# lionelblonde/sac-td3-cudagraphs-pytorch

Hardware: AMD Instinct MI355X
Metric: gradient-steps/sec (SAC, batch=256) at 1 GPU + 8-seed node; replay HBM GB/s (higher is better)
Workload: dtype f32; 1 GPU; SAC Hopper-v4 batch=256 2x256 MLP+LN, 100000 rows in a 1000000-row HBM ring, 1 critic update+Polyak per iteration, 2 actor+alpha updates every 3rd, hipGraph per 3 iterations; parallelism=1 independent seeds, one per GPU, no collective

## Files before the change

sac-td3-cudagraphs-pytorch_amd/csrc/kernels.h:

```cpp
#pragma once
#include <hip/hip_runtime.h>
#include <stddef.h>
#include <stdint.h>
#include <type_traits>
#include "philox.h"

#define HID 256
#define LN_EPS 1e-5f
#define NSLOT 5
#define AS 260
#define WS 68
#define YS 20

typedef float f32x4 __attribute__((ext_vector_type(4)));

#ifdef SACTD3_STAMPS
__device__ long long g_stamps[16];
__device__ long long g_phase[8];
#define PHASE_DECL long long ph_t = 0, ph_acc[6] = {0, 0, 0, 0, 0, 0}
#define PHASE_START do { __builtin_amdgcn_s_waitcnt(0xc07f); ph_t = clock64(); } while (0)
#define PHASE(i) do { const long long n_ = clock64(); ph_acc[i] += n_ - ph_t; ph_t = n_; } while (0)
#define PHASE_DRAIN(i) do { __builtin_amdgcn_s_waitcnt(0); const long long n_ = clock64(); ph_acc[i] += n_ - ph_t; ph_t = n_; } while (0)
#define PHASE_OUT do { if (threadIdx.x == 0 && blockIdx.x == gridDim.x - 1) for (int i_ = 0; i_ < 6; ++i_) g_phase[i_] = ph_acc[i_]; } while (0)
#define STAMP(i) do { if (threadIdx.x == 0 && blockIdx.x == gridDim.x - 1 && blockIdx.y == 0 && blockIdx.z == 0) { __builtin_amdgcn_s_waitcnt(0); g_stamps[i] = clock64(); } } while (0)
// ... 29 lines not shown
  int pad_seq;
  float metrics[8];
  float adam_q[2], adam_a[2];
  double pw_q[2], pw_a[2], pw_l[2];
  alignas(128) int predict_ctr;
  int predict_seq;
  int pad_acting[30];
};
static_assert(offsetof(DevCtl, predict_ctr) % 128 == 0 && sizeof(DevCtl) % 128 == 0, "acting words need a line of their own");

struct NetLayout {
  int K, ld1, nh;
  int W1, b1, g1, be1, W2, b2, g2, be2, Wh, bh;
  int size;
};

__device__ __forceinline__ unsigned fast_div(unsigned n, unsigned d, unsigned magic) { return magic ? __umulhi(n, magic) : n / d; }
__device__ __forceinline__ int small_div(int n, int d) {
  int q = (int)((float)n * __frcp_rn((float)d));
  const int r = n - q * d;
  if (r < 0) --q; else if (r >= d) ++q;
  return q;
}
__device__ __forceinline__ void xcd_tile(int b, int R, int C, int xr, int& tr, int& tc) {
  if (xr <= 0) { tr = small_div(b, C); tc = b - tr * C; return; }
  const int lr = __builtin_ctz((unsigned)xr), lc = 3 - lr;
  const int x = b & 7, j = b >> 3;
  const int cl = C >> lc, rl = R >> lr;
  const int gr = x >> lc, gc = x - (gr << lc);
  const int jr = small_div(j, cl);
  tr = gr * rl + jr; tc = gc * cl + (j - jr * cl);
}

__device__ __forceinline__ void adam_tick(int* t, double* pw, float* out, float lr, float b1, float b2) {
  const int tv = *t;
  double q0 = 0.0, q1 = 0.0;
  if (out) { q0 = pw[0]; q1 = pw[1]; }
  *t = tv + 1;
  if (out) {
    const double p1 = q0 * (double)b1, p2 = q1 * (double)b2;
    pw[0] = p1; pw[1] = p2;
    out[0] = (float)((double)lr / (1.0 - p1));
    out[1] = (float)sqrt(1.0 - p2);
  }
}
__device__ int g_sink_i[2];
__device__ double g_sink_d[2];
__device__ float g_sink_f[2];
__device__ __forceinline__ void tick_all(int* t0, int* t1, double* pw, float* out, float lr, float b1, float b2) {
  const bool pub = t0 != nullptr && out != nullptr;
  t0 = t0 ? t0 : g_sink_i; t1 = t1 ? t1 : g_sink_i + 1;
  pw = pub ? pw : g_sink_d; out = pub ? out : g_sink_f;
  const int a = *t0, b = *t1;
  const double q0 = pw[0], q1 = pw[1];
  const double p1 = q0 * (double)b1, p2 = q1 * (double)b2;
  *t0 = a + 1; *t1 = b + 1;
  pw[0] = p1; pw[1] = p2;
  out[0] = (float)((double)lr / (1.0 - p1));
  out[1] = (float)sqrt(1.0 - p2);
}
#define PIN(x) asm volatile("" : "+v"(x))
template <int CTRL> __device__ __forceinline__ float dpp_mov(float v) {
  return __builtin_bit_cast(float, __builtin_amdgcn_update_dpp(0, __builtin_bit_cast(int, v), CTRL, 0xF, 0xF, true));
}
__device__ __forceinline__ float row16_sum(float v) {
  v += dpp_mov<0xB1>(v);
  v += dpp_mov<0x4E>(v);
  v += dpp_mov<0x141>(v);
  v += dpp_mov<0x140>(v);
  return v;
}
__device__ __forceinline__ float lane_bcast(float v, int l) {
  return __builtin_bit_cast(float, __builtin_amdgcn_readlane(__builtin_bit_cast(int, v), l));
}
__device__ __forceinline__ float wave_sum(float v) {
  v = row16_sum(v);
  return (lane_bcast(v, 0) + lane_bcast(v, 16)) + (lane_bcast(v, 32) + lane_bcast(v, 48));
}
__device__ __forceinline__ float sum4(float4 v) { return (v.x + v.y) + (v.z + v.w); }
__device__ __forceinline__ float dot4(float4 a, float4 b) { return a.x * b.x + a.y * b.y + a.z * b.z + a.w * b.w; }
__device__ __forceinline__ float4 ld4(const float* p) { return *reinterpret_cast<const float4*>(p); }
__device__ __forceinline__ void st4(float* p, float4 v) { *reinterpret_cast<float4*>(p) = v; }
#ifndef SACTD3_WT
#define SACTD3_WT 1
#endif
constexpr bool WT_ACT1 = (SACTD3_WT & 1) != 0;
constexpr bool WT_Z2 = (SACTD3_WT & 2) != 0;
constexpr bool WT_DZ = (SACTD3_WT & 4) != 0;
typedef unsigned int u32x4 __attribute__((ext_vector_type(4)));
__device__ __forceinline__ void st4_wt(float* base, long off, float4 v) {
  const u32x4 u = {__float_as_uint(v.x), __float_as_uint(v.y), __float_as_uint(v.z), __float_as_uint(v.w)};
  __builtin_amdgcn_raw_buffer_store_b128(u, __builtin_amdgcn_make_buffer_rsrc(base, 0, 0x7fffffff, 0x00020000), (int)(4 * off), 0, 16);
}
__device__ __forceinline__ void st1_wt(float* p, float v) { __hip_atomic_store(p, v, __ATOMIC_RELAXED, __HIP_MEMORY_SCOPE_AGENT); }
template <bool WT> __device__ __forceinline__ void st4_pol(float* base, long off, float4 v) { if (WT) st4_wt(base, off, v); else st4(base + off, v); }
template <bool WT> __device__ __forceinline__ void st1_pol(float* p, float v) { if (WT) st1_wt(p, v); else *p = v; }
__device__ __forceinline__ float4 f4(float a) { return make_float4(a, a, a, a); }
__device__ __forceinline__ float4 operator+(float4 a, float4 b) { return make_float4(a.x + b.x, a.y + b.y, a.z + b.z, a.w + b.w); }
__device__ __forceinline__ float4 operator-(float4 a, float4 b) { return make_float4(a.x - b.x, a.y - b.y, a.z - b.z, a.w - b.w); }
__device__ __forceinline__ float4 operator*(float4 a, float4 b) { return make_float4(a.x * b.x, a.y * b.y, a.z * b.z, a.w * b.w); }
__device__ __forceinline__ float4 operator*(float4 a, float b) { return make_float4(a.x * b, a.y * b, a.z * b, a.w * b); }
__device__ __forceinline__ float4 relu4(float4 a) { return make_float4(fmaxf(a.x, 0.f), fmaxf(a.y, 0.f), fmaxf(a.z, 0.f), fmaxf(a.w, 0.f)); }
__device__ __forceinline__ float4 gate4(float4 v, float4 y) {
  return make_float4(y.x > 0.f ? v.x : 0.f, y.y > 0.f ? v.y : 0.f, y.z > 0.f ? v.z : 0.f, y.w > 0.f ? v.w : 0.f);
}
__device__ __forceinline__ float4 ld4_cols(const float* row, int k, int K, int Kr, bool row_ok = true) {
  const float4 v = ld4(row + min(k, Kr - 4));
  float4 o;
  o.x = (row_ok && k < K) ? v.x : 0.f;
  o.y = (row_ok && k + 1 < K) ? v.y : 0.f;
  o.z = (row_ok && k + 2 < K) ? v.z : 0.f;
  o.w = (row_ok && k + 3 < K) ? v.w : 0.f;
  return o;
}

__device__ __forceinline__ float4 ld4_raw(const float* row, int k, int Kr) { return ld4(row + min(k, Kr - 4)); }
__device__ __forceinline__ float4 mask4_cols(float4 v, int k, int K, bool row_ok = true) {
  float4 o;
  o.x = (row_ok && k < K) ? v.x : 0.f;
  o.y = (row_ok && k + 1 < K) ? v.y : 0.f;
  o.z = (row_ok && k + 2 < K) ? v.z : 0.f;
  o.w = (row_ok && k + 3 < K) ? v.w : 0.f;
  return o;
}

__device__ __forceinline__ float philox_normal(unsigned long long seed, unsigned ctr, unsigned site, unsigned e) {
  const Philox4 r = philox4x32_10(ctr, 0u, SACTD3_STREAM_NOISE + site, e >> 2, (uint32_t)seed, (uint32_t)(seed >> 32));
  const unsigned k = e & 3u;
  const float u1 = philox_u01((k & 2u) ? r.v[2] : r.v[0]), u2 = philox_u01((k & 2u) ? r.v[3] : r.v[1]);
  const float rad = sqrtf(-2.0f * 0.6931471805599453f * __builtin_amdgcn_logf(u1));
  return (k & 1u) ? rad * __builtin_amdgcn_sinf(u2) : rad * __builtin_amdgcn_cosf(u2);
}

__device__ __forceinline__ float4 philox_normal4(unsigned long long seed, unsigned ctr, unsigned site, unsigned q) {
  const Philox4 r = philox4x32_10(ctr, 0u, SACTD3_STREAM_NOISE + site, q, (uint32_t)seed, (uint32_t)(seed >> 32));
  const float ua = philox_u01(r.v[0]), ub = philox_u01(r.v[1]), uc = philox_u01(r.v[2]), ud = philox_u01(r.v[3]);
  const float r0 = sqrtf(-2.0f * 0.6931471805599453f * __builtin_amdgcn_logf(ua));
  const float r1 = sqrtf(-2.0f * 0.6931471805599453f * __builtin_amdgcn_logf(uc));
  return make_float4(r0 * __builtin_amdgcn_cosf(ub), r0 * __builtin_amdgcn_sinf(ub), r1 * __builtin_amdgcn_cosf(ud), r1 * __builtin_amdgcn_sinf(ud));
}
struct NoiseJob { float* eps; const int* ctr; int ctr_add; unsigned site_code; int site_buf; int n; int blocks; };
__device__ __forceinline__ void noise_body(const NoiseJob& z, const DevCtl* ctl, unsigned local_block) {
  const int inject = ctl->inject_eps[z.site_buf], ctr = *z.ctr;
  const unsigned long long seed = ctl->seed;
  const unsigned q = local_block * 256u + threadIdx.x;
  if (inject || 4 * q >= (unsigned)z.n) return;
  const float4 v = philox_normal4(seed, (unsigned)(ctr + z.ctr_add), z.site_code, q);
  float* d = z.eps + 4 * (long)q;
  d[0] = v.x;
  if (4 * q + 1 < (unsigned)z.n) d[1] = v.y;
  if (4 * q + 2 < (unsigned)z.n) d[2] = v.z;
  if (4 * q + 3 < (unsigned)z.n) d[3] = v.w;
}

struct Row16 { float4 v[4]; };
__device__ __forceinline__ Row16 row_ld(const float* row, int sub) {
  Row16 r;
#pragma unroll
  for (int q = 0; q < 4; ++q) r.v[q] = ld4(row + 4 * sub + 64 * q);
  return r;
}
__device__ __forceinline__ void row_pin(Row16& r) {
#pragma unroll
  for (int q = 0; q < 4; ++q) { PIN(r.v[q].x); PIN(r.v[q].y); PIN(r.v[q].z); PIN(r.v[q].w); }
}
__device__ __forceinline__ void row_st(float* row, int sub, const Row16& r) {
#pragma unroll
  for (int q = 0; q < 4; ++q) st4(row + 4 * sub + 64 * q, r.v[q]);
}
__device__ __forceinline__ float row_dot(const Row16& a, const Row16& b) {
  return (dot4(a.v[0], b.v[0]) + dot4(a.v[1], b.v[1])) + (dot4(a.v[2], b.v[2]) + dot4(a.v[3], b.v[3]));
}
__device__ __forceinline__ float row_total(const Row16& a) { return (sum4(a.v[0]) + sum4(a.v[1])) + (sum4(a.v[2]) + sum4(a.v[3])); }

__device__ __forceinline__ void ln_fwd(const Row16& z, const Row16& g, const Row16& be, int ln, Row16& xh, Row16& y, float& rstd) {
  if (ln) {
    const float mean = row16_sum(row_total(z)) * (1.0f / HID);
    Row16 d;
#pragma unroll
    for (int q = 0; q < 4; ++q) d.v[q] = z.v[q] - f4(mean);
    const float var = row16_sum(row_dot(d, d)) * (1.0f / HID);
    rstd = 1.0f / sqrtf(var + LN_EPS);
#pragma unroll
    for (int q = 0; q < 4; ++q) { xh.v[q] = d.v[q] * rstd; y.v[q] = xh.v[q] * g.v[q] + be.v[q]; }
  } else {
    rstd = 1.f; xh = z; y = z;
  }
}
__device__ __forceinline__ Row16 ln_bwd(const Row16& dy, const Row16& xh, float rstd, const Row16& g, int ln) {
  if (!ln) return dy;
  Row16 dxh, dz;
#pragma unroll
  for (int q = 0; q < 4; ++q) dxh.v[q] = dy.v[q] * g.v[q];
  const float m1 = row16_sum(row_total(dxh)) * (1.0f / HID);
  const float m2 = row16_sum(row_dot(dxh, xh)) * (1.0f / HID);
#pragma unroll
  for (int q = 0; q < 4; ++q) dz.v[q] = (dxh.v[q] - f4(m1) - xh.v[q] * m2) * rstd;
  return dz;
}
template <int RPB>
__device__ __forceinline__ void block_colsum(float* cs, const Row16* vals, int nslots, int row, int sub, float* dst) {
  for (int s = 0; s < nslots; ++s) row_st(cs + (s * RPB + row) * HID, sub, vals[s]);
  __syncthreads();
  for (int c = threadIdx.x; c < HID; c += 16 * RPB)
    for (int s = 0; s < nslots; ++s) {
      float a = 0.f;
#pragma unroll
      for (int r = 0; r < RPB; ++r) a += cs[(s * RPB + r) * HID + c];
      dst[s * HID + c] = a;
    }
}

struct GatherArgs {
  const float4* ring; int rec4;
  int cx, cn;
  const DevCtl* ctl; int* idx;
  float4* X; float4* Xn;
  float* rew; float* done;
  int B; int len_override;
  unsigned rec4_magic;
  int cpb;
  int ctr_add;
};

#ifndef GATHER_CPT
#define GATHER_CPT 4
#endif
__device__ __forceinline__ void gather_body(const GatherArgs& p, unsigned block) {
  __shared__ int ids_s[GATHER_CPT * 256 + 2];
  const int inject = p.ctl->inject_idx, rb_len = p.ctl->rb_len, ctr = p.ctl->sample_ctr + p.ctr_add;
  const unsigned long long seed = p.ctl->seed;
  const int len = p.len_override >= 0 ? p.len_override : rb_len;
  const unsigned total = (unsigned)p.B * (unsigned)p.rec4;
  const unsigned c0 = block * (unsigned)p.cpb * 256u;
  if (c0 >= total) return;
  const unsigned c1 = min(c0 + (unsigned)p.cpb * 256u, total);
// ... 1816 lines not shown
  const Row16 zo = row_ld(p.z2 + ((long)net * p.B + bc) * HID, sub);
  const Row16 wt0 = row_ld(p.PT + p.L.Wh, sub), wt1 = row_ld(p.PT + p.p_ns + p.L.Wh, sub), wo = row_ld(Pn + p.L.Wh, sub);
  Row16 gt0, bt0, gt1, bt1, go, bo;
  if (p.ln) {
    gt0 = row_ld(p.PT + p.L.g2, sub); bt0 = row_ld(p.PT + p.L.be2, sub);
    gt1 = row_ld(p.PT + p.p_ns + p.L.g2, sub); bt1 = row_ld(p.PT + p.p_ns + p.L.be2, sub);
    go = row_ld(Pn + p.L.g2, sub); bo = row_ld(Pn + p.L.be2, sub);
  }
  const float bht0 = p.PT[p.L.bh], bht1 = p.PT[p.p_ns + p.L.bh], bho = Pn[p.L.bh];
  const float rw = p.rew[bc], dn = p.done[bc];
  const float alpha = p.sac ? expf(*p.log_alpha) : 0.f;
  const float lpn = p.sac ? p.logp_next[bc] : 0.f;
  STAMP(1);
  Row16 xh, y, h; float rs;
  ln_fwd(zt0, gt0, bt0, p.ln, xh, y, rs);
#pragma unroll
  for (int q = 0; q < 4; ++q) h.v[q] = relu4(y.v[q]);
  const float qt0 = row16_sum(row_dot(h, wt0)) + bht0;
  ln_fwd(zt1, gt1, bt1, p.ln, xh, y, rs);
#pragma unroll
  for (int q = 0; q < 4; ++q) h.v[q] = relu4(y.v[q]);
  const float qt1 = row16_sum(row_dot(h, wt1)) + bht1;
  const float qmin = fminf(qt0, qt1);
  float qp = p.bcq ? 0.75f * qmin + 0.25f * fmaxf(qt0, qt1) : qmin;
  if (p.sac) qp -= alpha * lpn;
  const float yv = rw + (1.0f - dn) * p.gamma * qp;
  float rstd;
  ln_fwd(zo, go, bo, p.ln, xh, y, rstd);
#pragma unroll
  for (int q = 0; q < 4; ++q) h.v[q] = relu4(y.v[q]);
  const float qv = row16_sum(row_dot(h, wo)) + bho;
  const float err = valid ? qv - yv : 0.f;
  const float dq = 2.0f * err / (float)p.B;
  Row16 dy, vals[3];
#pragma unroll
  for (int q = 0; q < 4; ++q) dy.v[q] = gate4(wo.v[q] * dq, y.v[q]);
  const Row16 dz = ln_bwd(dy, xh, rstd, go, p.ln);
#pragma unroll
  for (int q = 0; q < 4; ++q) { vals[0].v[q] = dy.v[q] * xh.v[q]; vals[1].v[q] = dy.v[q]; vals[2].v[q] = h.v[q] * dq; }
  if (valid) {
    row_st(p.dz2 + ((long)net * p.B + b) * HID, sub, dz);
    if (sub == 0) {
      p.q[(long)net * p.B + b] = qv;
      if (net == 0) { p.qt[b] = qt0; p.qt[p.B + b] = qt1; p.y[b] = yv; }
    }
  }
  if (sub == 0) { sc[row][0] = dq; sc[row][1] = err * err; }
  STAMP(2);
  const long blk = (long)net * p.pstride + blockIdx.x;
  block_colsum<RPB>(cs, vals, 3, row, sub, p.part + blk * NSLOT * HID);
  if (t < 2) {
    float s = 0.f;
#pragma unroll
    for (int i = 0; i < RPB; ++i) s += sc[i][t];
    p.part_s[blk * 2 + t] = s;
  }
  STAMP(3);
}

struct NnFold { int fold, ln; const float* h1; const float* xh1; int g1_off; float* ps; float* gsnap; };
struct CtailNn { CriticTail c; const float* Wt; int ldw; float* dX; int xr; NnFold f; };
__device__ __forceinline__ void nn_fold_store(const NnFold& f, const float* o, const float* hv, const float* xv, float gcol,
                                              float* x, float* ps, float* gsnap, int row0, int B, int col, int lane) {
  if (f.fold && f.ln && row0 == 0 && lane < 16) gsnap[col] = gcol;
#pragma unroll
  for (int i = 0; i < 4; ++i) {
    const int orow = row0 + 4 * (lane >> 4) + i;
    const float dy = f.fold ? (hv[i] > 0.f ? o[i] : 0.f) : o[i];
    if (orow < B) x[(long)orow * HID + col] = dy;
    if (f.fold && f.ln) {
      const float dxh = dy * gcol;
      const float s1 = row16_sum(dxh), s2 = row16_sum(dxh * xv[i]);
      if ((lane & 15) == 0 && orow < B) { ps[(long)orow * PS_W + (col >> 4)] = s1; ps[(long)orow * PS_W + 16 + (col >> 4)] = s2; }
    }
  }
}
template <int NT>
__global__ __launch_bounds__(256) void k_ctail_nn(CtailNn a) {
  const CriticTail& p = a.c;
  constexpr int CB = 16 * NT;
  __shared__ __attribute__((aligned(16))) float Dz[16 * AS];
  __shared__ __attribute__((aligned(16))) float cs[3 * 16 * CB];
  __shared__ __attribute__((aligned(16))) float red[NT * 4 * 64 * 4];
  __shared__ float sc[16][2];
  const int t = threadIdx.x, lane = t & 63, wave = t >> 6, row = t >> 4, sub = t & 15, net = blockIdx.z;
  const int r = lane & 15, kq = lane >> 4;
  int tm, tk;
  xcd_tile(blockIdx.x, (p.B + 15) >> 4, HID / CB, a.xr, tm, tk);
  const int b = tm * 16 + row, bc = min(b, p.B - 1), c_lo = tk * CB;
  const bool valid = b < p.B;
  const float* Pn = p.P + net * p.p_ns;
  const Row16 zt0 = row_ld(p.z2t + (long)bc * HID, sub), zt1 = row_ld(p.z2t + ((long)p.B + bc) * HID, sub);
  const Row16 zo = row_ld(p.z2 + ((long)net * p.B + bc) * HID, sub);
  const Row16 wt0 = row_ld(p.PT + p.L.Wh, sub), wt1 = row_ld(p.PT + p.p_ns + p.L.Wh, sub), wo = row_ld(Pn + p.L.Wh, sub);
  Row16 gt0, bt0, gt1, bt1, go, bo;
  if (p.ln) {
    gt0 = row_ld(p.PT + p.L.g2, sub); bt0 = row_ld(p.PT + p.L.be2, sub);
    gt1 = row_ld(p.PT + p.p_ns + p.L.g2, sub); bt1 = row_ld(p.PT + p.p_ns + p.L.be2, sub);
    go = row_ld(Pn + p.L.g2, sub); bo = row_ld(Pn + p.L.be2, sub);
  }
  const float bht0 = p.PT[p.L.bh], bht1 = p.PT[p.p_ns + p.L.bh], bho = Pn[p.L.bh];
  const float rw = p.rew[bc], dn = p.done[bc];
  const float alpha = p.sac ? expf(*p.log_alpha) : 0.f;
  const float lpn = p.sac ? p.logp_next[bc] : 0.f;
  const int nb = 64 * wave + 4 * kq;
  float4 bv[NT][4];
#pragma unroll
  for (int nt = 0; nt < NT; ++nt) {
    const float* Wc = a.Wt + net * p.p_ns + (long)nb * a.ldw + c_lo + 16 * nt + r;
#pragma unroll
    for (int c = 0; c < 4; ++c) {
      const float* w = Wc + (long)(16 * c) * a.ldw;
      bv[nt][c] = make_float4(w[0], w[a.ldw], w[2 * (long)a.ldw], w[3 * (long)a.ldw]);
    }
  }
  float fh[4] = {1.f, 1.f, 1.f, 1.f}, fx[4] = {0.f, 0.f, 0.f, 0.f}, fg = 1.f;
  if (a.f.fold && wave < NT) {
    const int col = c_lo + 16 * wave + (lane & 15);
#pragma unroll
    for (int i = 0; i < 4; ++i) {
      const long o = ((long)net * p.B + min(tm * 16 + 4 * (lane >> 4) + i, p.B - 1)) * HID + col;
      fh[i] = a.f.h1[o]; if (a.f.ln) fx[i] = a.f.xh1[o];
    }
    if (a.f.ln) fg = Pn[a.f.g1_off + col];
  }
  __builtin_amdgcn_sched_barrier(0);
  Row16 xh, y, h; float rs;
  ln_fwd(zt0, gt0, bt0, p.ln, xh, y, rs);
#pragma unroll
  for (int q = 0; q < 4; ++q) h.v[q] = relu4(y.v[q]);
  const float qt0 = row16_sum(row_dot(h, wt0)) + bht0;
  ln_fwd(zt1, gt1, bt1, p.ln, xh, y, rs);
#pragma unroll
  for (int q = 0; q < 4; ++q) h.v[q] = relu4(y.v[q]);
  const float qt1 = row16_sum(row_dot(h, wt1)) + bht1;
  const float qmin = fminf(qt0, qt1);
  float qp = p.bcq ? 0.75f * qmin + 0.25f * fmaxf(qt0, qt1) : qmin;
  if (p.sac) qp -= alpha * lpn;
  const float yv = rw + (1.0f - dn) * p.gamma * qp;
  float rstd;
  ln_fwd(zo, go, bo, p.ln, xh, y, rstd);
#pragma unroll
  for (int q = 0; q < 4; ++q) h.v[q] = relu4(y.v[q]);
  const float qv = row16_sum(row_dot(h, wo)) + bho;
  const float err = valid ? qv - yv : 0.f;
  const float dq = 2.0f * err / (float)p.B;
  Row16 dy, vals[3];
#pragma unroll
  for (int q = 0; q < 4; ++q) dy.v[q] = gate4(wo.v[q] * dq, y.v[q]);
  const Row16 dz = ln_bwd(dy, xh, rstd, go, p.ln);
#pragma unroll
  for (int q = 0; q < 4; ++q) { vals[0].v[q] = dy.v[q] * xh.v[q]; vals[1].v[q] = dy.v[q]; vals[2].v[q] = h.v[q] * dq; }
#pragma unroll
  for (int nt = 0; nt < NT; ++nt)
#pragma unroll
    for (int c = 0; c < 4; ++c) { PIN(bv[nt][c].x); PIN(bv[nt][c].y); PIN(bv[nt][c].z); PIN(bv[nt][c].w); }
  row_st(Dz + row * AS, sub, dz);
#pragma unroll
  for (int q = 0; q < 4; ++q) {
    const int col = 4 * sub + 64 * q;
    if (col >= c_lo && col < c_lo + CB) {
      if (valid) st4_pol<WT_DZ>(p.dz2, ((long)net * p.B + b) * HID + col, dz.v[q]);
#pragma unroll
      for (int sl = 0; sl < 3; ++sl) st4(cs + (sl * 16 + row) * CB + (col - c_lo), vals[sl].v[q]);
    }
  }
  if (tk == 0 && sub == 0) {
    sc[row][0] = dq; sc[row][1] = err * err;
    if (valid) {
      p.q[(long)net * p.B + b] = qv;
      if (net == 0) { p.qt[b] = qt0; p.qt[p.B + b] = qt1; p.y[b] = yv; }
    }
  }
  __syncthreads();
  const long blk = (long)net * p.pstride + tm;
  if (t < 3 * CB) {
    const int sl = t / CB, c = t - sl * CB;
    float sum = 0.f;
#pragma unroll
    for (int i = 0; i < 16; ++i) sum += cs[(sl * 16 + i) * CB + c];
    p.part[(blk * NSLOT + sl) * HID + c_lo + c] = sum;
  }
  if (tk == 0 && t >= 128 && t < 130) {
    float sum = 0.f;
#pragma unroll
    for (int i = 0; i < 16; ++i) sum += sc[i][t - 128];
    p.part_s[blk * 2 + (t - 128)] = sum;
  }
  f32x4 acc[NT];
#pragma unroll
  for (int nt = 0; nt < NT; ++nt) acc[nt] = f32x4{0.f, 0.f, 0.f, 0.f};
#pragma unroll
  for (int c = 0; c < 4; ++c) {
    const float4 av = ld4(Dz + r * AS + nb + 16 * c);
#pragma unroll
    for (int nt = 0; nt < NT; ++nt) { MFMA4(acc[nt], av, bv[nt][c]); }
  }
#pragma unroll
  for (int nt = 0; nt < NT; ++nt) st4(red + ((nt * 4 + wave) * 64 + lane) * 4, make_float4(acc[nt][0], acc[nt][1], acc[nt][2], acc[nt][3]));
  __syncthreads();
  if (wave < NT) {
    const float* rr = red + (wave * 4 * 64 + lane) * 4;
    const float4 x0 = ld4(rr), x1 = ld4(rr + 256), x2 = ld4(rr + 512), x3 = ld4(rr + 768);
    const float o[4] = {(x0.x + x1.x) + (x2.x + x3.x), (x0.y + x1.y) + (x2.y + x3.y), (x0.z + x1.z) + (x2.z + x3.z), (x0.w + x1.w) + (x2.w + x3.w)};
    const int col = c_lo + 16 * wave + (lane & 15);
    nn_fold_store(a.f, o, fh, fx, fg, a.dX + (long)net * p.B * HID, a.f.ps + (long)net * p.B * PS_W, a.f.gsnap + net * HID, tm * 16, p.B, col, lane);
  }
}

struct ActorQTail {
  const float* z2c;
  const float* P; long p_ns; NetLayout L;
  const float* logp; const float* log_alpha;
  int B, ln, sac;
  float* q; float* dz2;
  float* part_s;
};

template <int RPB>
__global__ __launch_bounds__(16 * RPB) void k_actorq_tail(ActorQTail p) {
  __shared__ float sc[RPB];
  const int t = threadIdx.x, row = t >> 4, sub = t & 15;
  const int b = blockIdx.x * RPB + row, bc = min(b, p.B - 1);
  const bool valid = b < p.B;
  const int nq = p.sac ? 2 : 1;
  Row16 z[2], w[2], g[2], be[2], xh[2], y[2];
  float rstd[2], qv[2] = {0.f, 0.f}, bh[2];
#pragma unroll
  for (int i = 0; i < 2; ++i)
    if (i < nq) {
      const float* Pn = p.P + i * p.p_ns;
      z[i] = row_ld(p.z2c + ((long)i * p.B + bc) * HID, sub);
      w[i] = row_ld(Pn + p.L.Wh, sub);
      if (p.ln) { g[i] = row_ld(Pn + p.L.g2, sub); be[i] = row_ld(Pn + p.L.be2, sub); }
      bh[i] = Pn[p.L.bh];
    }
  const float alpha = p.sac ? expf(*p.log_alpha) : 0.f;
  const float lpv = p.sac ? p.logp[bc] : 0.f;
#pragma unroll
  for (int i = 0; i < 2; ++i)
    if (i < nq) {
      ln_fwd(z[i], g[i], be[i], p.ln, xh[i], y[i], rstd[i]);
      Row16 h;
#pragma unroll
      for (int q = 0; q < 4; ++q) h.v[q] = relu4(y[i].v[q]);
      qv[i] = row16_sum(row_dot(h, w[i])) + bh[i];
    }
  const bool first = p.sac ? (qv[0] <= qv[1]) : true;
  const float loss = p.sac ? (alpha * lpv - (first ? qv[0] : qv[1])) : -qv[0];
  const float invB = 1.0f / (float)p.B;
#pragma unroll
  for (int i = 0; i < 2; ++i)
    if (i < nq) {
      const float dq = ((i == 0) == first) ? -invB : 0.f;
      Row16 dy;
#pragma unroll
      for (int q = 0; q < 4; ++q) dy.v[q] = gate4(w[i].v[q] * dq, y[i].v[q]);
      const Row16 dz = ln_bwd(dy, xh[i], rstd[i], g[i], p.ln);
      if (valid) {
        row_st(p.dz2 + ((long)i * p.B + b) * HID, sub, dz);
        if (sub == 0) p.q[(long)i * p.B + b] = qv[i];
      }
    }
  if (sub == 0) sc[row] = valid ? loss : 0.f;
  __syncthreads();
  if (t == 0) {
    float s = 0.f;
#pragma unroll
    for (int i = 0; i < RPB; ++i) s += sc[i];
    p.part_s[blockIdx.x * 2 + 1] = s;
  }
}

struct QaFold {
  int on, ln, a, pqw, ntile;
  const float* h1; const float* xh1;
  int g1_off, w1_off, ld1, k_off;
  float* ps;
  float* S;
};
struct QtailNn { ActorQTail c; const float* Wt; int ldw; float* dX; int xr; QaFold qa; };
template <int NT>
__global__ __launch_bounds__(256) void k_qtail_nn(QtailNn a) {
  const ActorQTail& p = a.c;
  constexpr int CB = 16 * NT;
  __shared__ __attribute__((aligned(16))) float Dz[16 * AS];
  __shared__ __attribute__((aligned(16))) float red[NT * 4 * 64 * 4];
  __shared__ float sc[16];
  const int t = threadIdx.x, lane = t & 63, wave = t >> 6, row = t >> 4, sub = t & 15, net = blockIdx.z;
  const int r = lane & 15, kq = lane >> 4;
  int tm, tk;
  xcd_tile(blockIdx.x, (p.B + 15) >> 4, HID / CB, a.xr, tm, tk);
  const int b = tm * 16 + row, bc = min(b, p.B - 1), c_lo = tk * CB;
  const bool valid = b < p.B;
  const int nq = p.sac ? 2 : 1;
  Row16 z[2], w[2], g[2], be[2], xh[2], y[2];
  float rstd[2], qv[2] = {0.f, 0.f}, bh[2];
#pragma unroll
  for (int i = 0; i < 2; ++i)
    if (i < nq) {
      const float* Pi = p.P + i * p.p_ns;
      z[i] = row_ld(p.z2c + ((long)i * p.B + bc) * HID, sub);
      w[i] = row_ld(Pi + p.L.Wh, sub);
      if (p.ln) { g[i] = row_ld(Pi + p.L.g2, sub); be[i] = row_ld(Pi + p.L.be2, sub); }
      bh[i] = Pi[p.L.bh];
    }
  const float alpha = p.sac ? expf(*p.log_alpha) : 0.f;
  const float lpv = p.sac ? p.logp[bc] : 0.f;
  const int nb = 64 * wave + 4 * kq;
  float4 bv[NT][4];
#pragma unroll
  for (int nt = 0; nt < NT; ++nt) {
    const float* Wc = a.Wt + net * p.p_ns + (long)nb * a.ldw + c_lo + 16 * nt + r;
#pragma unroll
    for (int c = 0; c < 4; ++c) {
      const float* wp = Wc + (long)(16 * c) * a.ldw;
      bv[nt][c] = make_float4(wp[0], wp[a.ldw], wp[2 * (long)a.ldw], wp[3 * (long)a.ldw]);
    }
  }
  float qh[NT][4], qx[NT][4], qg[NT];
  float4 qw[NT];
#pragma unroll
  for (int nt = 0; nt < NT; ++nt) {
    qg[nt] = 1.f; qw[nt] = f4(0.f);
#pragma unroll
    for (int i = 0; i < 4; ++i) { qh[nt][i] = 1.f; qx[nt][i] = 0.f; }
  }
  if (a.qa.on && wave == 0) {
    const float* Pn = p.P + net * p.p_ns;
#pragma unroll
    for (int nt = 0; nt < NT; ++nt) {
      const int col = c_lo + 16 * nt + (lane & 15);
#pragma unroll
      for (int i = 0; i < 4; ++i) {
        const long o = ((long)net * p.B + min(tm * 16 + 4 * (lane >> 4) + i, p.B - 1)) * HID + col;
        qh[nt][i] = a.qa.h1[o]; if (a.qa.ln) qx[nt][i] = a.qa.xh1[o];
      }
      if (a.qa.ln) qg[nt] = Pn[a.qa.g1_off + col];
      const float* wr = Pn + a.qa.w1_off + (long)(c_lo + 16 * nt + 4 * kq) * a.qa.ld1 + a.qa.k_off + min(r, a.qa.a - 1);
      qw[nt] = make_float4(wr[0], wr[a.qa.ld1], wr[2 * (long)a.qa.ld1], wr[3 * (long)a.qa.ld1]);
    }
  }
  __builtin_amdgcn_sched_barrier(0);
#pragma unroll
  for (int i = 0; i < 2; ++i)
    if (i < nq) {
      ln_fwd(z[i], g[i], be[i], p.ln, xh[i], y[i], rstd[i]);
      Row16 h;
#pragma unroll
      for (int q = 0; q < 4; ++q) h.v[q] = relu4(y[i].v[q]);
      qv[i] = row16_sum(row_dot(h, w[i])) + bh[i];
    }
  const bool first = p.sac ? (qv[0] <= qv[1]) : true;
  const float loss = p.sac ? (alpha * lpv - (first ? qv[0] : qv[1])) : -qv[0];
  const float invB = 1.0f / (float)p.B;
  const bool mine = valid && ((net == 0) == first);
  const float dq = mine ? -invB : 0.f;
  Row16 dy;
  const Row16& wn = net == 0 ? w[0] : w[1];
  const Row16& yn = net == 0 ? y[0] : y[1];
  const Row16& xn = net == 0 ? xh[0] : xh[1];
  const Row16& gn = net == 0 ? g[0] : g[1];
#pragma unroll
  for (int q = 0; q < 4; ++q) dy.v[q] = gate4(wn.v[q] * dq, yn.v[q]);
  const Row16 dz = ln_bwd(dy, xn, net == 0 ? rstd[0] : rstd[1], gn, p.ln);
#pragma unroll
  for (int nt = 0; nt < NT; ++nt)
#pragma unroll
    for (int c = 0; c < 4; ++c) { PIN(bv[nt][c].x); PIN(bv[nt][c].y); PIN(bv[nt][c].z); PIN(bv[nt][c].w); }
  row_st(Dz + row * AS, sub, dz);
  if (tk == 0 && sub == 0) {
    if (valid) p.q[(long)net * p.B + b] = net == 0 ? qv[0] : qv[1];
    if (net == 0) sc[row] = valid ? loss : 0.f;
  }
  __syncthreads();
  if (tk == 0 && net == 0 && t == 0) {
    float sum = 0.f;
#pragma unroll
    for (int i = 0; i < 16; ++i) sum += sc[i];
    p.part_s[tm * 2 + 1] = sum;
  }
  f32x4 acc[NT];
#pragma unroll
  for (int nt = 0; nt < NT; ++nt) acc[nt] = f32x4{0.f, 0.f, 0.f, 0.f};
#pragma unroll
  for (int c = 0; c < 4; ++c) {
    const float4 av = ld4(Dz + r * AS + nb + 16 * c);
#pragma unroll
    for (int nt = 0; nt < NT; ++nt) { MFMA4(acc[nt], av, bv[nt][c]); }
  }
#pragma unroll
  for (int nt = 0; nt < NT; ++nt) st4(red + ((nt * 4 + wave) * 64 + lane) * 4, make_float4(acc[nt][0], acc[nt][1], acc[nt][2], acc[nt][3]));
  __syncthreads();
  if (a.qa.on) {
    if (wave != 0) return;
    const int na = a.qa.a;
    f32x4 aP = {0.f, 0.f, 0.f, 0.f}, aX = {0.f, 0.f, 0.f, 0.f}, aS = {0.f, 0.f, 0.f, 0.f};
    float s2r[4] = {0.f, 0.f, 0.f, 0.f};
#pragma unroll
    for (int nt = 0; nt < NT; ++nt) {
      float* T = red + nt * 4 * 64 * 4;
      const float4 x0 = ld4(T + lane * 4), x1 = ld4(T + 256 + lane * 4), x2 = ld4(T + 512 + lane * 4), x3 = ld4(T + 768 + lane * 4);
      const float o[4] = {(x0.x + x1.x) + (x2.x + x3.x), (x0.y + x1.y) + (x2.y + x3.y), (x0.z + x1.z) + (x2.z + x3.z), (x0.w + x1.w) + (x2.w + x3.w)};
      float4 bw = qw[nt];
      if (r >= na) bw = f4(r == na ? 1.f : 0.f);
      __builtin_amdgcn_s_waitcnt(0xc07f);
#pragma unroll
      for (int i = 0; i < 4; ++i) {
        const float dy = qh[nt][i] > 0.f ? o[i] : 0.f;
        const float dxh = a.qa.ln ? dy * qg[nt] : dy;
        if (a.qa.ln) s2r[i] += row16_sum(dxh * qx[nt][i]);
        T[(4 * (lane >> 4) + i) * 20 + (lane & 15)] = dxh;
        T[320 + (4 * (lane >> 4) + i) * 20 + (lane & 15)] = qx[nt][i];
      }
      const float4 fa = ld4(T + r * 20 + 4 * kq), fx4 = ld4(T + 320 + r * 20 + 4 * kq);
      MFMA4(aP, fa, bw);
      if (a.qa.ln) { MFMA4(aX, fx4, bw); }
      if (a.qa.ln && tm == 0) { const float4 one = f4(1.f); MFMA4(aS, one, bw); }
    }
    float* ps = a.qa.ps + (((long)net * p.B) * a.qa.ntile + tk) * a.qa.pqw;
#pragma unroll
    for (int i = 0; i < 4; ++i) {
      const int orow = tm * 16 + 4 * (lane >> 4) + i;
      if (orow >= p.B) continue;
      float* d = ps + (long)orow * a.qa.ntile * a.qa.pqw;
      if (r <= na) d[r] = aP[i];
// ... 190 lines not shown
  const Row16 dz = ln_bwd(dy, xh, rstd, g, p.ln);
  if (valid) row_st(p.dz2 + (long)b * HID, sub, dz);
#pragma unroll
  for (int q = 0; q < 4; ++q) { vals[0].v[q] = dy.v[q] * xh.v[q]; vals[1].v[q] = dy.v[q]; }
  block_colsum<16>(cs, vals, 2, row, sub, p.part + (long)blockIdx.x * NSLOT * HID);
}

template <int RPB>
__global__ __launch_bounds__(16 * RPB) void k_actor_head_bwd_s(ActorHeadBwd p) {
  __shared__ __attribute__((aligned(16))) float cs[2 * RPB * HID];
  const int t = threadIdx.x, row = t >> 4, sub = t & 15;
  const int b = blockIdx.x * RPB + row, bc = min(b, p.B - 1);
  const bool valid = b < p.B;
  const int nh = p.L.nh;
  const float* Wh = p.P + p.L.Wh;
  const long ro = (long)bc * HID;
  const Row16 hh = row_ld(p.h2 + ro, sub), xh = row_ld(p.xh2 + ro, sub);
  Row16 g;
  if (p.ln) g = row_ld(p.P + p.L.g2, sub);
  const float rstd = p.ln ? p.rstd2[bc] : 1.f;
  Row16 w[8];
#pragma unroll
  for (int n = 0; n < 8; ++n) w[n] = row_ld(Wh + (long)min(n, nh - 1) * HID, sub);
  const bool second = sub >= p.a;
  const int j0 = min(second ? sub - p.a : sub, p.a - 1);
  const float* tgr = p.tg + (long)bc * 4 * p.a4;
  float la = p.sac ? *p.log_alpha : 0.f;
  float o_dA = p.dA[(long)bc * p.ldA + j0], o_dA1 = p.nq == 2 ? p.dA[p.dA_ns + (long)bc * p.ldA + j0] : 0.f;
  float o_sc = p.scale[j0], o_t0 = tgr[j0];
  float o_t1 = 0.f, o_t2 = 0.f, o_e = 0.f;
  if (p.sac) { o_t1 = tgr[p.a4 + j0]; o_t2 = tgr[2 * p.a4 + j0]; o_e = p.eps[(long)bc * p.a + j0]; }
  PIN(la); PIN(o_dA); PIN(o_dA1); PIN(o_sc); PIN(o_t0); PIN(o_t1); PIN(o_t2); PIN(o_e);
  const float dlogp = p.sac ? expf(la) / (float)p.B : 0.f;
  float d;
  {
    const float dAj = o_dA + o_dA1, sc = o_sc;
    float g_mean, g_raw = 0.f;
    if (p.sac) {
      const float tt = o_t0, sd = o_t1, yt = o_t2;
      const float omy2 = 1.0f - yt * yt;
      const float g0 = dAj * sc * omy2 + dlogp * (2.0f * sc * yt * omy2) / (sc * omy2 + 1e-6f);
      g_mean = g0;
      g_raw = (g0 * o_e * sd - dlogp) * 3.5f * (1.0f - tt * tt);
    } else {
      g_mean = dAj * sc * (1.0f - o_t0 * o_t0);
    }
    d = second ? g_raw : g_mean;
    if (!valid || sub >= nh) d = 0.f;
  }
  Row16 dh;
#pragma unroll
  for (int q = 0; q < 4; ++q) dh.v[q] = f4(0.f);
  auto add_n = [&](float dn, const Row16& wn) {
#pragma unroll
    for (int q = 0; q < 4; ++q) dh.v[q] = dh.v[q] + wn.v[q] * dn;
  };
  row_pin(w[0]); add_n(dpp_mov<0x150>(d), w[0]);
  row_pin(w[1]); add_n(dpp_mov<0x151>(d), w[1]);
  row_pin(w[2]); add_n(dpp_mov<0x152>(d), w[2]);
  row_pin(w[3]); add_n(dpp_mov<0x153>(d), w[3]);
  row_pin(w[4]); add_n(dpp_mov<0x154>(d), w[4]);
  row_pin(w[5]); add_n(dpp_mov<0x155>(d), w[5]);
  row_pin(w[6]); add_n(dpp_mov<0x156>(d), w[6]);
  row_pin(w[7]); add_n(dpp_mov<0x157>(d), w[7]);
  if (valid && sub < nh) p.du[(long)b * p.ldu + sub] = d;
  Row16 dy, vals[2];
#pragma unroll
  for (int q = 0; q < 4; ++q) dy.v[q] = gate4(dh.v[q], hh.v[q]);
  const Row16 dz = ln_bwd(dy, xh, rstd, g, p.ln);
  if (valid) row_st(p.dz2 + (long)b * HID, sub, dz);
#pragma unroll
  for (int q = 0; q < 4; ++q) { vals[0].v[q] = dy.v[q] * xh.v[q]; vals[1].v[q] = dy.v[q]; }
  block_colsum<RPB>(cs, vals, 2, row, sub, p.part + (long)blockIdx.x * NSLOT * HID);
}

struct QaIn { int on, ln, a, pqw, ntile; const float* ps; const float* S; const float* rstd; float* dA; };
struct HeadBwdNn { ActorHeadBwd c; const float* Wt; int ldw; float* dX; int xr; NnFold f; QaIn qa; };
__global__ __launch_bounds__(256) void k_headbwd_nn(HeadBwdNn a) {
  const ActorHeadBwd& p = a.c;
  constexpr int CB = 16;
  __shared__ __attribute__((aligned(16))) float Dz[16 * AS];
  __shared__ __attribute__((aligned(16))) float cs[2 * 16 * CB];
  __shared__ __attribute__((aligned(16))) float red[4 * 64 * 4];
  const int t = threadIdx.x, lane = t & 63, wave = t >> 6, row = t >> 4, sub = t & 15;
  const int r = lane & 15, kq = lane >> 4;
  int tm, tk;
  xcd_tile(blockIdx.x, (p.B + 15) >> 4, HID / CB, a.xr, tm, tk);
  const int b = tm * 16 + row, bc = min(b, p.B - 1), c_lo = tk * CB;
  const bool valid = b < p.B;
  const int nh = p.L.nh;
  const float* Wh = p.P + p.L.Wh;
  const long ro = (long)bc * HID;
  const Row16 hh = row_ld(p.h2 + ro, sub), xh = row_ld(p.xh2 + ro, sub);
  Row16 g;
  if (p.ln) g = row_ld(p.P + p.L.g2, sub);
  const float rstd = p.ln ? p.rstd2[bc] : 1.f;
  Row16 w[8];
#pragma unroll
  for (int n = 0; n < 8; ++n) w[n] = row_ld(Wh + (long)min(n, nh - 1) * HID, sub);
  const bool second = sub >= p.a;
  const int j0 = min(second ? sub - p.a : sub, p.a - 1);
  const float* tgr = p.tg + (long)bc * 4 * p.a4;
  float la = p.sac ? *p.log_alpha : 0.f;
  float o_dA = 0.f, o_dA1 = 0.f;
  float4 qv[2] = {f4(0.f), f4(0.f)}, qs[2] = {f4(0.f), f4(0.f)};
  float qrs[2] = {1.f, 1.f};
  if (a.qa.on) {
    const int n4 = a.qa.ntile * a.qa.pqw / 4, s4 = a.qa.ntile * 2;
#pragma unroll
    for (int q = 0; q < 2; ++q)
      if (q < p.nq) {
        const float* pr = a.qa.ps + ((long)q * p.B + bc) * (long)n4 * 4;
        float4 v0 = ld4(pr + 4 * sub), v1 = f4(0.f), v2 = f4(0.f), v3 = f4(0.f);
        if (n4 > 16) v1 = ld4(pr + 4 * (sub + 16));
        if (n4 > 32) { v2 = ld4(pr + 4 * (sub + 32)); v3 = ld4(pr + 4 * (sub + 48)); }
        qv[q] = (v0 + v1) + (v2 + v3);
        const float* sr = a.qa.S + (long)q * s4 * 4;
        float4 t0 = ld4(sr + 4 * sub), t1 = f4(0.f);
        if (s4 > 16) t1 = ld4(sr + 4 * (sub + 16));
        qs[q] = t0 + t1;
        if (a.qa.ln) qrs[q] = a.qa.rstd[(long)q * p.B + bc];
      }
  } else {
    o_dA = p.dA[(long)bc * p.ldA + j0]; o_dA1 = p.nq == 2 ? p.dA[p.dA_ns + (long)bc * p.ldA + j0] : 0.f;
  }
  float o_sc = p.scale[j0], o_t0 = tgr[j0];
  float o_t1 = 0.f, o_t2 = 0.f, o_e = 0.f;
  if (p.sac) { o_t1 = tgr[p.a4 + j0]; o_t2 = tgr[2 * p.a4 + j0]; o_e = p.eps[(long)bc * p.a + j0]; }
  const int nb = 64 * wave + 4 * kq;
  float4 bv[4];
  {
    const float* Wc = a.Wt + (long)nb * a.ldw + c_lo + r;
#pragma unroll
    for (int c = 0; c < 4; ++c) {
      const float* wp = Wc + (long)(16 * c) * a.ldw;
      bv[c] = make_float4(wp[0], wp[a.ldw], wp[2 * (long)a.ldw], wp[3 * (long)a.ldw]);
    }
  }
  float fh[4] = {1.f, 1.f, 1.f, 1.f}, fx[4] = {0.f, 0.f, 0.f, 0.f}, fg = 1.f;
  if (a.f.fold && wave == 0) {
    const int col = c_lo + (lane & 15);
#pragma unroll
    for (int i = 0; i < 4; ++i) {
      const long o = (long)min(tm * 16 + 4 * (lane >> 4) + i, p.B - 1) * HID + col;
      fh[i] = a.f.h1[o]; if (a.f.ln) fx[i] = a.f.xh1[o];
    }
    if (a.f.ln) fg = p.P[a.f.g1_off + col];
  }
  __builtin_amdgcn_sched_barrier(0);
  if (a.qa.on) {
    float* Vs = red + (row * 2) * 24;
#pragma unroll
    for (int q = 0; q < 2; ++q)
      if (q < p.nq) {
        float v[8] = {qv[q].x, qv[q].y, qv[q].z, qv[q].w, qs[q].x, qs[q].y, qs[q].z, qs[q].w};
#pragma unroll
        for (int k = 0; k < 8; ++k) {
          if (k >= 4 || a.qa.pqw == 8) v[k] += dpp_mov<0x122>(v[k]);
          v[k] += dpp_mov<0x124>(v[k]); v[k] += dpp_mov<0x128>(v[k]);
        }
        if (sub < a.qa.pqw / 4) st4(Vs + q * 24 + 4 * sub, make_float4(v[0], v[1], v[2], v[3]));
        if (sub < 2) st4(Vs + q * 24 + 16 + 4 * sub, make_float4(v[4], v[5], v[6], v[7]));
      }
    const int na = a.qa.a;
    float tot = 0.f;
#pragma unroll
    for (int q = 0; q < 2; ++q)
      if (q < p.nq) {
        const float* V = Vs + q * 24;
        const float P = V[j0];
        float dq = P;
        if (a.qa.ln) dq = (P - V[na] * (1.0f / HID) * V[16 + j0] - V[2 * na + 1] * (1.0f / HID) * V[na + 1 + j0]) * qrs[q];
        if (a.qa.dA && tk == 0 && valid && sub < na) a.qa.dA[((long)q * p.B + b) * p.ldA + sub] = dq;
        tot += dq;
      }
    o_dA = tot; o_dA1 = 0.f;
  }
  PIN(la); PIN(o_dA); PIN(o_dA1); PIN(o_sc); PIN(o_t0); PIN(o_t1); PIN(o_t2); PIN(o_e);
  const float dlogp = p.sac ? expf(la) / (float)p.B : 0.f;
  float d;
  {
    const float dAj = o_dA + o_dA1, sc = o_sc;
    float g_mean, g_raw = 0.f;
    if (p.sac) {
      const float tt = o_t0, sd = o_t1, yt = o_t2;
      const float omy2 = 1.0f - yt * yt;
      const float g0 = dAj * sc * omy2 + dlogp * (2.0f * sc * yt * omy2) / (sc * omy2 + 1e-6f);
      g_mean = g0;
      g_raw = (g0 * o_e * sd - dlogp) * 3.5f * (1.0f - tt * tt);
    } else {
      g_mean = dAj * sc * (1.0f - o_t0 * o_t0);
    }
    d = second ? g_raw : g_mean;
    if (!valid || sub >= nh) d = 0.f;
  }
  Row16 dh;
#pragma unroll
  for (int q = 0; q < 4; ++q) dh.v[q] = f4(0.f);
  auto add_n = [&](float dn, const Row16& wn) {
#pragma unroll
    for (int q = 0; q < 4; ++q) dh.v[q] = dh.v[q] + wn.v[q] * dn;
  };
  row_pin(w[0]); add_n(dpp_mov<0x150>(d), w[0]);
  row_pin(w[1]); add_n(dpp_mov<0x151>(d), w[1]);
  row_pin(w[2]); add_n(dpp_mov<0x152>(d), w[2]);
  row_pin(w[3]); add_n(dpp_mov<0x153>(d), w[3]);
  row_pin(w[4]); add_n(dpp_mov<0x154>(d), w[4]);
  row_pin(w[5]); add_n(dpp_mov<0x155>(d), w[5]);
  row_pin(w[6]); add_n(dpp_mov<0x156>(d), w[6]);
  row_pin(w[7]); add_n(dpp_mov<0x157>(d), w[7]);
#pragma unroll
  for (int c = 0; c < 4; ++c) { PIN(bv[c].x); PIN(bv[c].y); PIN(bv[c].z); PIN(bv[c].w); }
  if (tk == 0 && valid && sub < nh) p.du[(long)b * p.ldu + sub] = d;
  Row16 dy, vals[2];
#pragma unroll
  for (int q = 0; q < 4; ++q) dy.v[q] = gate4(dh.v[q], hh.v[q]);
  const Row16 dz = ln_bwd(dy, xh, rstd, g, p.ln);
#pragma unroll
  for (int q = 0; q < 4; ++q) { vals[0].v[q] = dy.v[q] * xh.v[q]; vals[1].v[q] = dy.v[q]; }
  row_st(Dz + row * AS, sub, dz);
#pragma unroll
  for (int q = 0; q < 4; ++q) {
    const int col = 4 * sub + 64 * q;
    if (col >= c_lo && col < c_lo + CB) {
      if (valid) st4_pol<WT_DZ>(p.dz2, (long)b * HID + col, dz.v[q]);
#pragma unroll
      for (int sl = 0; sl < 2; ++sl) st4(cs + (sl * 16 + row) * CB + (col - c_lo), vals[sl].v[q]);
    }
  }
  __syncthreads();
  if (t < 2 * CB) {
    const int sl = t / CB, c = t - sl * CB;
// ... 71 lines not shown
```

Before: 19570 gradient-steps/s.

## Stage head weight/LN vectors through LDS in critic-tail and actor head kernels

```diff
diff --git a/sac-td3-cudagraphs-pytorch_amd/csrc/kernels.h b/sac-td3-cudagraphs-pytorch_amd/csrc/kernels.h
--- a/sac-td3-cudagraphs-pytorch_amd/csrc/kernels.h
+++ b/sac-td3-cudagraphs-pytorch_amd/csrc/kernels.h
@@ -135,7 +135,7 @@
 __device__ __forceinline__ float4 ld4(const float* p) { return *reinterpret_cast<const float4*>(p); }
 __device__ __forceinline__ void st4(float* p, float4 v) { *reinterpret_cast<float4*>(p) = v; }
 #ifndef SACTD3_WT
-#define SACTD3_WT 1
+#define SACTD3_WT 5
 #endif
 constexpr bool WT_ACT1 = (SACTD3_WT & 1) != 0;
 constexpr bool WT_Z2 = (SACTD3_WT & 2) != 0;
@@ -205,6 +205,12 @@
   if (4 * q + 2 < (unsigned)z.n) d[2] = v.z;
   if (4 * q + 3 < (unsigned)z.n) d[3] = v.w;
 }
+
+#ifndef SACTD3_TP
+#define SACTD3_TP 1
+#endif
+constexpr bool TP_PARK = (SACTD3_TP & 1) != 0;
+constexpr int TP_NV = 9;
 
 struct Row16 { float4 v[4]; };
 __device__ __forceinline__ Row16 row_ld(const float* row, int sub) {
@@ -2187,6 +2193,7 @@
   __shared__ __attribute__((aligned(16))) float Dz[16 * AS];
   __shared__ __attribute__((aligned(16))) float cs[3 * 16 * CB];
   __shared__ __attribute__((aligned(16))) float red[NT * 4 * 64 * 4];
+  __shared__ __attribute__((aligned(16))) float Pv[TP_PARK ? TP_NV * HID + 4 : 4];
   __shared__ float sc[16][2];
   const int t = threadIdx.x, lane = t & 63, wave = t >> 6, row = t >> 4, sub = t & 15, net = blockIdx.z;
   const int r = lane & 15, kq = lane >> 4;
@@ -2195,16 +2202,27 @@
   const int b = tm * 16 + row, bc = min(b, p.B - 1), c_lo = tk * CB;
   const bool valid = b < p.B;
   const float* Pn = p.P + net * p.p_ns;
+  const int kind = p.ln ? min(wave, 2) : 0;
+  const bool parks = TP_PARK && wave == kind;
+  float4 pa, pb, pc; float pbh;
+  if (TP_PARK) {
+    const int ko = (kind == 0 ? p.L.Wh : kind == 1 ? p.L.g2 : p.L.be2) + 4 * lane;
+    pa = ld4(p.PT + ko); pb = ld4(p.PT + p.p_ns + ko); pc = ld4(Pn + ko);
+    pbh = (lane == 0 ? p.PT : lane == 1 ? p.PT + p.p_ns : Pn)[p.L.bh];
+  }
   const Row16 zt0 = row_ld(p.z2t + (long)bc * HID, sub), zt1 = row_ld(p.z2t + ((long)p.B + bc) * HID, sub);
   const Row16 zo = row_ld(p.z2 + ((long)net * p.B + bc) * HID, sub);
-  const Row16 wt0 = row_ld(p.PT + p.L.Wh, sub), wt1 = row_ld(p.PT + p.p_ns + p.L.Wh, sub), wo = row_ld(Pn + p.L.Wh, sub);
-  Row16 gt0, bt0, gt1, bt1, go, bo;
-  if (p.ln) {
-    gt0 = row_ld(p.PT + p.L.g2, sub); bt0 = row_ld(p.PT + p.L.be2, sub);
-    gt1 = row_ld(p.PT + p.p_ns + p.L.g2, sub); bt1 = row_ld(p.PT + p.p_ns + p.L.be2, sub);
-    go = row_ld(Pn + p.L.g2, sub); bo = row_ld(Pn + p.L.be2, sub);
-  }
-  const float bht0 = p.PT[p.L.bh], bht1 = p.PT[p.p_ns + p.L.bh], bho = Pn[p.L.bh];
+  Row16 wt0, wt1, wo, gt0, bt0, gt1, bt1, go, bo;
+  float bht0 = 0.f, bht1 = 0.f, bho = 0.f;
+  if (!TP_PARK) {
+    wt0 = row_ld(p.PT + p.L.Wh, sub); wt1 = row_ld(p.PT + p.p_ns + p.L.Wh, sub); wo = row_ld(Pn + p.L.Wh, sub);
+    if (p.ln) {
+      gt0 = row_ld(p.PT + p.L.g2, sub); bt0 = row_ld(p.PT + p.L.be2, sub);
+      gt1 = row_ld(p.PT + p.p_ns + p.L.g2, sub); bt1 = row_ld(p.PT + p.p_ns + p.L.be2, sub);
+      go = row_ld(Pn + p.L.g2, sub); bo = row_ld(Pn + p.L.be2, sub);
+    }
+    bht0 = p.PT[p.L.bh]; bht1 = p.PT[p.p_ns + p.L.bh]; bho = Pn[p.L.bh];
+  }
   const float rw = p.rew[bc], dn = p.done[bc];
   const float alpha = p.sac ? expf(*p.log_alpha) : 0.f;
   const float lpn = p.sac ? p.logp_next[bc] : 0.f;
@@ -2230,11 +2248,25 @@
     if (a.f.ln) fg = Pn[a.f.g1_off + col];
   }
   __builtin_amdgcn_sched_barrier(0);
+  if (TP_PARK) {
+    if (parks) { st4(Pv + kind * HID + 4 * lane, pa); st4(Pv + (3 + kind) * HID + 4 * lane, pb); st4(Pv + (6 + kind) * HID + 4 * lane, pc); }
+    if (wave == 3 && lane < 3) Pv[TP_NV * HID + lane] = pbh;
+    __syncthreads();
+    bht0 = Pv[TP_NV * HID]; bht1 = Pv[TP_NV * HID + 1]; bho = Pv[TP_NV * HID + 2];
+  }
+  auto net_vecs = [&](int n, Row16& wn, Row16& gn, Row16& bn) {
+    if (!TP_PARK) return;
+    if (n) __builtin_amdgcn_sched_barrier(0);
+    wn = row_ld(Pv + 3 * n * HID, sub);
+    if (p.ln) { gn = row_ld(Pv + (3 * n + 1) * HID, sub); bn = row_ld(Pv + (3 * n + 2) * HID, sub); }
+  };
   Row16 xh, y, h; float rs;
+  net_vecs(0, wt0, gt0, bt0);
   ln_fwd(zt0, gt0, bt0, p.ln, xh, y, rs);
 #pragma unroll
   for (int q = 0; q < 4; ++q) h.v[q] = relu4(y.v[q]);
   const float qt0 = row16_sum(row_dot(h, wt0)) + bht0;
+  net_vecs(1, wt1, gt1, bt1);
   ln_fwd(zt1, gt1, bt1, p.ln, xh, y, rs);
 #pragma unroll
   for (int q = 0; q < 4; ++q) h.v[q] = relu4(y.v[q]);
@@ -2244,6 +2276,7 @@
   if (p.sac) qp -= alpha * lpn;
   const float yv = rw + (1.0f - dn) * p.gamma * qp;
   float rstd;
+  net_vecs(2, wo, go, bo);
   ln_fwd(zo, go, bo, p.ln, xh, y, rstd);
 #pragma unroll
   for (int q = 0; q < 4; ++q) h.v[q] = relu4(y.v[q]);
@@ -2391,6 +2424,7 @@
   constexpr int CB = 16 * NT;
   __shared__ __attribute__((aligned(16))) float Dz[16 * AS];
   __shared__ __attribute__((aligned(16))) float red[NT * 4 * 64 * 4];
+  __shared__ __attribute__((aligned(16))) float Pv[TP_PARK ? 6 * HID + 4 : 4];
   __shared__ float sc[16];
   const int t = threadIdx.x, lane = t & 63, wave = t >> 6, row = t >> 4, sub = t & 15, net = blockIdx.z;
   const int r = lane & 15, kq = lane >> 4;
@@ -2400,15 +2434,25 @@
   const bool valid = b < p.B;
   const int nq = p.sac ? 2 : 1;
   Row16 z[2], w[2], g[2], be[2], xh[2], y[2];
-  float rstd[2], qv[2] = {0.f, 0.f}, bh[2];
+  float rstd[2], qv[2] = {0.f, 0.f}, bh[2] = {0.f, 0.f};
+  const int kind = p.ln ? min(wave, 2) : 0;
+  const bool parks = TP_PARK && wave == kind;
+  float4 pa, pb; float pbh;
+  if (TP_PARK) {
+    const int ko = (kind == 0 ? p.L.Wh : kind == 1 ? p.L.g2 : p.L.be2) + 4 * lane;
+    pa = ld4(p.P + ko); pb = ld4(p.P + (nq - 1) * p.p_ns + ko);
+    pbh = p.P[(long)min(lane, nq - 1) * p.p_ns + p.L.bh];
+  }
 #pragma unroll
   for (int i = 0; i < 2; ++i)
     if (i < nq) {
       const float* Pi = p.P + i * p.p_ns;
       z[i] = row_ld(p.z2c + ((long)i * p.B + bc) * HID, sub);
-      w[i] = row_ld(Pi + p.L.Wh, sub);
-      if (p.ln) { g[i] = row_ld(Pi + p.L.g2, sub); be[i] = row_ld(Pi + p.L.be2, sub); }
-      bh[i] = Pi[p.L.bh];
+      if (!TP_PARK) {
+        w[i] = row_ld(Pi + p.L.Wh, sub);
+        if (p.ln) { g[i] = row_ld(Pi + p.L.g2, sub); be[i] = row_ld(Pi + p.L.be2, sub); }
+        bh[i] = Pi[p.L.bh];
+      }
     }
   const float alpha = p.sac ? expf(*p.log_alpha) : 0.f;
   const float lpv = p.sac ? p.logp[bc] : 0.f;
@@ -2447,6 +2491,18 @@
     }
   }
   __builtin_amdgcn_sched_barrier(0);
+  if (TP_PARK) {
+    if (parks) { st4(Pv + kind * HID + 4 * lane, pa); if (nq == 2) st4(Pv + (3 + kind) * HID + 4 * lane, pb); }
+    if (wave == 3 && lane < nq) Pv[6 * HID + lane] = pbh;
+    __syncthreads();
+#pragma unroll
+    for (int i = 0; i < 2; ++i)
+      if (i < nq) {
+        w[i] = row_ld(Pv + 3 * i * HID, sub);
+        if (p.ln) { g[i] = row_ld(Pv + (3 * i + 1) * HID, sub); be[i] = row_ld(Pv + (3 * i + 2) * HID, sub); }
+        bh[i] = Pv[6 * HID + i];
+      }
+  }
 #pragma unroll
   for (int i = 0; i < 2; ++i)
     if (i < nq) {
@@ -2803,6 +2859,7 @@
   __shared__ __attribute__((aligned(16))) float Dz[16 * AS];
   __shared__ __attribute__((aligned(16))) float cs[2 * 16 * CB];
   __shared__ __attribute__((aligned(16))) float red[4 * 64 * 4];
+  __shared__ __attribute__((aligned(16))) float Pv[TP_PARK ? TP_NV * HID : 4];
   const int t = threadIdx.x, lane = t & 63, wave = t >> 6, row = t >> 4, sub = t & 15;
   const int r = lane & 15, kq = lane >> 4;
   int tm, tk;
@@ -2812,13 +2869,21 @@
   const int nh = p.L.nh;
   const float* Wh = p.P + p.L.Wh;
   const long ro = (long)bc * HID;
+  float4 pa, pb, pc;
+  if (TP_PARK) {
+    pa = ld4(Wh + (long)min(wave, nh - 1) * HID + 4 * lane);
+    pb = ld4(Wh + (long)min(wave + 4, nh - 1) * HID + 4 * lane);
+    if (p.ln) pc = ld4(p.P + p.L.g2 + 4 * lane);
+  }
   const Row16 hh = row_ld(p.h2 + ro, sub), xh = row_ld(p.xh2 + ro, sub);
   Row16 g;
-  if (p.ln) g = row_ld(p.P + p.L.g2, sub);
+  if (!TP_PARK && p.ln) g = row_ld(p.P + p.L.g2, sub);
   const float rstd = p.ln ? p.rstd2[bc] : 1.f;
   Row16 w[8];
-#pragma unroll
-  for (int n = 0; n < 8; ++n) w[n] = row_ld(Wh + (long)min(n, nh - 1) * HID, sub);
+  if (!TP_PARK) {
+#pragma unroll
+    for (int n = 0; n < 8; ++n) w[n] = row_ld(Wh + (long)min(n, nh - 1) * HID, sub);
+  }
   const bool second = sub >= p.a;
   const int j0 = min(second ? sub - p.a : sub, p.a - 1);
   const float* tgr = p.tg + (long)bc * 4 * p.a4;
@@ -2869,6 +2934,15 @@
     if (a.f.ln) fg = p.P[a.f.g1_off + col];
   }
   __builtin_amdgcn_sched_barrier(0);
+  if (TP_PARK) {
+    if (wave < nh) st4(Pv + wave * HID + 4 * lane, pa);
+    if (wave + 4 < nh) st4(Pv + (wave + 4) * HID + 4 * lane, pb);
+    if (p.ln && wave == 3) st4(Pv + 8 * HID + 4 * lane, pc);
+    __syncthreads();
+    if (p.ln) g = row_ld(Pv + 8 * HID, sub);
+#pragma unroll
+    for (int n = 0; n < 8; ++n) w[n] = row_ld(Pv + min(n, nh - 1) * HID, sub);
+  }
   if (a.qa.on) {
     float* Vs = red + (row * 2) * 24;
 #pragma unroll
```

New measurement: 19720 gradient-steps/s, median of 2. Within noise of the previous version (+0.7%).
